# taaha-khan/2023-CompaCT-Image-Compression

Hardware: AMD Instinct MI355X
Metric: MPixels/s encode+decode, 12-bit 512x512 CT batch, bytes-exact (higher is better)
Workload: dtype u16

## Files before the change

### 2023-compact-image-compression_amd/csrc/deflate_kernels.hip

```cpp
#include <hip/hip_runtime.h>
#include <cstring>
#include <algorithm>

#include "cct_internal.h"
#include "wave_device.h"
#include "../../include/compact_hip.h"

namespace cct {
namespace {

constexpr int MIN_MATCH = 3, MAX_MATCH = 258, WSIZE = 32768;
constexpr int MIN_LOOKAHEAD = MAX_MATCH + MIN_MATCH + 1;
constexpr int MAX_DIST = WSIZE - MIN_LOOKAHEAD;
constexpr int TOO_FAR = 4096;
constexpr int BLOCK_SYMS = 16383;
constexpr int BLOCK_SYMS_ML9 = 32767;
constexpr int L_CODES = 286, D_CODES = 30, BL_CODES = 19, HEAP_SIZE = 2 * L_CODES + 1;
constexpr int END_BLOCK = 256, MAX_BITS = 15, MAX_BL_BITS = 7;
constexpr uint32_t Z_FILTERED = 1, Z_HUFFMAN_ONLY = 2, Z_RLE = 3, Z_FIXED = 4;
__host__ __device__ __forceinline__ bool short_pass(uint32_t strategy) { return strategy == Z_HUFFMAN_ONLY || strategy == Z_RLE; }

__constant__ uint8_t c_extra_lbits[29] = {0,0,0,0,0,0,0,0,1,1,1,1,2,2,2,2,3,3,3,3,4,4,4,4,5,5,5,5,0};
__constant__ uint8_t c_extra_dbits[30] = {0,0,0,0,1,1,2,2,3,3,4,4,5,5,6,6,7,7,8,8,9,9,10,10,11,11,12,12,13,13};
__constant__ uint8_t c_extra_blbits[19] = {0,0,0,0,0,0,0,0,0,0,0,0,0,0,0,0,2,3,7};
__constant__ uint8_t c_bl_order[19] = {16,17,18,0,8,7,9,6,10,5,11,4,12,3,13,2,14,1,15};
__constant__ uint8_t c_length_code[256];
__constant__ uint16_t c_base_length[29];
__constant__ uint8_t c_dist_code[512];
__constant__ uint16_t c_base_dist[30];
__constant__ uint16_t c_static_lcode[288];
__constant__ uint8_t c_static_llen[288];
__constant__ uint16_t c_static_dcode[30];

template <int HB>
__device__ __forceinline__ uint32_t hash3(uint32_t b0, uint32_t b1, uint32_t b2)
{
	constexpr int SH = (HB + 2) / 3;
	return ((b0 << (2 * SH)) ^ (b1 << SH) ^ b2) & ((1u << HB) - 1u);
}

__device__ __forceinline__ int d_code(uint32_t dist) { return dist < 256 ? c_dist_code[dist] : c_dist_code[256 + (dist >> 7)]; }

struct MatchRec { uint16_t len_full, len_quarter, dist_full, dist_quarter; };
constexpr uint32_t GEN_MAX = 16383;
__device__ __forceinline__ uint2 pack_match(uint32_t len_full, uint32_t len_quarter, uint32_t dist_full, uint32_t dist_quarter, uint32_t gen)
{
	return make_uint2((len_full | ((gen & 127u) << 9)) | ((len_quarter | ((gen >> 7) << 9)) << 16), dist_full | (dist_quarter << 16));
}
__device__ __forceinline__ MatchRec checked_match(MatchRec r, uint32_t gen, uint32_t rw, uint32_t p, uint32_t L)
{
	const uint32_t tag = (uint32_t)(r.len_full >> 9) | ((uint32_t)(r.len_quarter >> 9) << 7);
	const uint32_t lookahead = L - min(p, L);
	const uint32_t max_len = lookahead < (uint32_t)MAX_MATCH ? lookahead : (uint32_t)MAX_MATCH;
	const bool maximal = (rw >> 15) && (rw & 0x7FFFu) >= max_len && p + 2 < L;
	MatchRec o;
	const bool ok = tag == gen;
	o.len_full = ok ? (uint16_t)(r.len_full & 511u) : (uint16_t)(maximal ? max_len : 0u);
	o.len_quarter = ok ? (uint16_t)(r.len_quarter & 511u) : (uint16_t)(maximal ? max_len : 0u);
	o.dist_full = ok ? r.dist_full : (uint16_t)(maximal ? 1u : 0u);
	o.dist_quarter = ok ? r.dist_quarter : (uint16_t)(maximal ? 1u : 0u);
	return o;
}

template <bool FIRST, int HB>
__global__ void __launch_bounds__(1024) dfl_sort_pass_kernel(DeflateArgs a)
{
	constexpr int BITS = FIRST ? 8 : HB - 8, NB = 1 << BITS;
	constexpr uint32_t HMASK = (1u << HB) - 1u;
	__shared__ uint32_t offs[256];
	__shared__ uint32_t wcnt[16][NB];
	const int s = blockIdx.x;
	const uint32_t L = a.in_sizes[s];
	const uint8_t *in = a.in + (size_t)s * a.in_stride;
	const size_t base = (size_t)s * a.in_stride;
	const uint32_t npos = L >= MIN_MATCH ? L - 2 : 0;
	const uint64_t *rec_src = a.rec_in + base;
	uint64_t *rec_dst = (FIRST ? a.rec_in : a.rec_out) + base;
	const int tid = threadIdx.x, lane = tid & 63, wave = tid >> 6;
	const uint64_t lt_mask = (1ull << lane) - 1ull;
	if (tid < 256) offs[tid] = 0;
	__syncthreads();
	if (tid < NB) offs[tid] = a.sort_hist[(size_t)s * SORT_HIST + (FIRST ? 0 : 256) + tid];
	__syncthreads();
	if (wave == 0) {
		uint32_t v[4], sum = 0;
#pragma unroll
		for (int k = 0; k < 4; k++) { v[k] = offs[lane * 4 + k]; sum += v[k]; }
		uint32_t run = wave_incl_scan(sum) - sum;
#pragma unroll
		for (int k = 0; k < 4; k++) { offs[lane * 4 + k] = run; run += v[k]; }
	}
	__syncthreads();
#ifndef CCT_SORT_E
#define CCT_SORT_E 4
#endif
	constexpr int E = CCT_SORT_E;
	constexpr int ND = E / 4;
	const uint32_t last = npos ? npos - 1 : 0;
	static_assert(E % 4 == 0 && ND + 1 <= E, "pass A: whole dwords per lane, kept in ra[0 .. ND]");
#ifdef CCT_SORT_PROBE
	const bool compact = false;
#else
	const bool compact = HB == 15 && a.pos_mask != 0xFFFFFFFFu;
#endif
	const uint32_t dmax = (uint32_t)a.in_stride - 4u;
	auto fetch = [&](uint32_t tile_base, uint32_t (&ra)[E], uint32_t (&rb)[E]) {
		if (FIRST) {
#pragma unroll
			for (int d = 0; d < ND; d++) ra[d] = *reinterpret_cast<const uint32_t *>(in + min(tile_base + 256u * d + 4u * (uint32_t)lane, dmax));
			ra[ND] = *reinterpret_cast<const uint32_t *>(in + min(tile_base + 256u * ND, dmax));
#pragma unroll
			for (int e = 0; e < E; e++) rb[e] = compact ? a.run_len[base + min(tile_base + (uint32_t)(e * 64 + lane), last)] : 0u;
		} else {
#pragma unroll
			for (int e = 0; e < E; e++) {
				const uint64_t r = rec_src[min(tile_base + (uint32_t)(e * 64 + lane), last)];
				ra[e] = (uint32_t)r; rb[e] = (uint32_t)(r >> 32);
			}
		}
	};
	auto finish = [&](uint32_t tile_base, const uint32_t (&ra)[E], const uint32_t (&rb)[E], uint32_t (&h)[E], uint32_t (&p)[E]) {
#pragma unroll
		for (int e = 0; e < E; e++) {
			const uint32_t idx = tile_base + (uint32_t)(e * 64 + lane);
			if (FIRST) {
				const int la = (e & 3) * 16 + (lane >> 2);
				const uint32_t da = (uint32_t)__builtin_amdgcn_ds_bpermute(la << 2, (int)ra[e >> 2]);
				uint32_t db = (uint32_t)__builtin_amdgcn_ds_bpermute(((la + 1) & 63) << 2, (int)ra[e >> 2]);
				if ((e & 3) == 3) {
					const uint32_t nxt = (e >> 2) + 1 < ND ? (uint32_t)__builtin_amdgcn_readfirstlane((int)ra[(e >> 2) + 1 < ND ? (e >> 2) + 1 : 0]) : ra[ND];
					if (la == 63) db = nxt;
				}
				const uint32_t sh = (uint32_t)lane & 3u;
				const uint32_t w = __builtin_amdgcn_alignbyte(db, da, sh);
				const uint32_t b0 = w & 255u, b1 = (w >> 8) & 255u, b2 = (w >> 16) & 255u;
				h[e] = hash3<HB>(b0, b1, b2); p[e] = idx;
				if (compact) {
					const uint32_t b4 = (db >> (8u * sh)) & 255u;
					const uint32_t f16 = (b0 == b1 && b1 == b2) ? rb[e] : ((w >> 24) | (b4 << 8));
					h[e] |= (f16 << 15) | ((b0 >> 7) << 31); p[e] |= (b1 << 22) | (((b0 >> 5) & 3u) << 30);
				}
			}
			else { h[e] = rb[e]; p[e] = ra[e]; }
			if (idx >= npos) { h[e] = 0; p[e] = idx; }
		}
	};
	uint32_t hn[E], pn[E];
	{
		uint32_t ra[E], rb[E];
		fetch((uint32_t)(wave * 64 * E), ra, rb);
		finish((uint32_t)(wave * 64 * E), ra, rb, hn, pn);
	}
	for (uint32_t t0 = 0; t0 < npos; t0 += 1024 * E) {
		uint32_t h[E], p[E], rk[E], ra[E], rb[E];
		const uint32_t idx0 = t0 + (uint32_t)(wave * 64 * E + lane);
#pragma unroll
		for (int e = 0; e < E; e++) { h[e] = hn[e]; p[e] = pn[e]; }
		const uint32_t next_base = t0 + (uint32_t)(1024 * E + wave * 64 * E);
		fetch(next_base, ra, rb);
		for (int k = lane; k < NB; k += 64) wcnt[wave][k] = 0;
#pragma unroll
		for (int e = 0; e < E; e++) {
			const bool valid = idx0 + e * 64 < npos;
			const uint32_t d = FIRST ? (h[e] & 255u) : ((h[e] & HMASK) >> 8);
			uint64_t same = __ballot(valid);
#pragma unroll
			for (int b = 0; b < BITS; b++) {
				const bool bit = (d >> b) & 1u;
				const uint64_t bal = __ballot(bit);
				same &= bit ? bal : ~bal;
			}
			const uint32_t rank = (uint32_t)__popcll(same & lt_mask);
			uint32_t before = 0;
			if (valid) {
				before = wcnt[wave][d];
				if (rank == 0) wcnt[wave][d] = before + (uint32_t)__popcll(same);
			}
			rk[e] = before + rank;
		}
		lds_barrier();
		if (tid < NB) {
			uint32_t c[16], run = offs[tid];
#pragma unroll
			for (int w = 0; w < 16; w++) c[w] = wcnt[w][tid];
#pragma unroll
			for (int w = 0; w < 16; w++) { wcnt[w][tid] = run; run += c[w]; }
			offs[tid] = run;
		}
		lds_barrier();
#pragma unroll
		for (int e = 0; e < E; e++) asm volatile("" : "+v"(ra[e]), "+v"(rb[e]) :: "memory");
		finish(next_base, ra, rb, hn, pn);
#pragma unroll
		for (int e = 0; e < E; e++) {
			if (idx0 + e * 64 < npos) {
				const uint32_t d = FIRST ? (h[e] & 255u) : ((h[e] & HMASK) >> 8);
				const uint32_t dst = wcnt[wave][d] + rk[e];
				rec_dst[dst] = (uint64_t)p[e] | ((uint64_t)h[e] << 32);
			}
		}
	}
}

constexpr int LIGHT_STEPS = 12;

__device__ __forceinline__ bool xcd_slice(int n, int &s, uint32_t &part, uint32_t &nparts)
{
	const uint32_t lin = blockIdx.x + gridDim.x * blockIdx.y;
	const uint32_t c = lin & 7u, k = lin >> 3;
	nparts = gridDim.x;
	s = (int)(8u * (k / nparts) + c);
	part = k % nparts;
	return s < n;
}

__device__ __forceinline__ uint32_t nil_candidate(uint32_t p, uint32_t lookahead)
{
	return (lookahead < (uint32_t)MIN_LOOKAHEAD && p >= 32506u + 32768u && (p - 32506u) % 32768u == 0) ? p - 32506u : 0xFFFFFFFFu;
}


template <bool SORT, int HB>
__global__ void __launch_bounds__(256) dfl_run_len_kernel(DeflateArgs a)
{
	constexpr int NH = 256 + (1 << (HB - 8));
	__shared__ uint32_t wtot[4];
	__shared__ uint32_t hist[SORT ? NH : 1];
	if (SORT) for (int t = threadIdx.x; t < NH; t += 256) hist[t] = 0;
	__syncthreads();
	const int s = blockIdx.y;
	const uint32_t L = a.in_sizes[s];
	const uint8_t *in = a.in + (size_t)s * a.in_stride;
	uint16_t *rl = a.run_len + (size_t)s * a.in_stride;
	const int lane = threadIdx.x & 63, wave = threadIdx.x >> 6;
	const uint32_t nchunks = (L + RUNLEN_OUT - 1) / RUNLEN_OUT;
	for (uint32_t c = blockIdx.x; c < nchunks; c += gridDim.x) {
		const uint32_t c0 = c * RUNLEN_OUT;
		const uint32_t g = c0 + threadIdx.x * 8;
		uint8_t b[12];
		if (g + 12 <= L && g >= 1) {
			uint64_t w;
			__builtin_memcpy(&w, in + g, 8);
#pragma unroll
			for (int k = 0; k < 8; k++) b[k + 1] = (uint8_t)(w >> (8 * k));
			b[0] = in[g - 1];
			uint32_t w2; __builtin_memcpy(&w2, in + g + 8, 4);
			b[9] = (uint8_t)w2; b[10] = (uint8_t)(w2 >> 8); b[11] = (uint8_t)(w2 >> 16);
		} else {
#pragma unroll
			for (int k = 0; k < 12; k++) { const int64_t y = (int64_t)g - 1 + k; b[k] = (y >= 0 && y < (int64_t)L) ? in[y] : 0; }
		}
		if (SORT) {
			uint32_t hk[8], cnt = 0, h0 = 0;
			bool same = true;
#pragma unroll
			for (int k = 0; k < 8; k++) {
				const bool v = threadIdx.x * 8 + k < (uint32_t)RUNLEN_OUT && g + k + 2 < L;
				hk[k] = v ? hash3<HB>(b[k + 1], b[k + 2], b[k + 3]) : 0xFFFFFFFFu;
				if (v) { if (!cnt) h0 = hk[k]; else same &= hk[k] == h0; cnt++; }
			}
			const bool wave_same = __all(same && cnt == 8 && h0 == (uint32_t)__builtin_amdgcn_readfirstlane((int)h0));
			if (wave_same) {
				if (lane == 0) { atomicAdd(&hist[h0 & 255u], 512u); atomicAdd(&hist[256u + (h0 >> 8)], 512u); }
			} else if (same) {
				if (cnt) { atomicAdd(&hist[h0 & 255u], cnt); atomicAdd(&hist[256u + (h0 >> 8)], cnt); }
			} else {
#pragma unroll
				for (int k = 0; k < 8; k++)
					if (hk[k] != 0xFFFFFFFFu) { atomicAdd(&hist[hk[k] & 255u], 1u); atomicAdd(&hist[256u + (hk[k] >> 8)], 1u); }
			}
		}
		uint32_t chg = 0;
#pragma unroll
		for (int k = 0; k < 8; k++) chg |= (uint32_t)(b[k + 1] != b[k + 2] || g + k + 1 >= L) << k;
		uint32_t hc = chg != 0, n = hc ? (uint32_t)__ffs((int)chg) - 1u : 8u;
#pragma unroll
		for (int d = 1; d < 64; d <<= 1) {
			const uint32_t hb = (uint32_t)__shfl_down((int)hc, d, 64), nb = (uint32_t)__shfl_down((int)n, d, 64);
			if (lane + d < 64 && !hc) { n += nb; hc = hb; }
		}
		__syncthreads();
		if (lane == 0) wtot[wave] = (hc << 31) | n;
		__syncthreads();
// ... 538 lines not shown
				nxt = p + k + (uint32_t)len;
				cnt = k + 1;
			}
		}
		a.rec32[base + p] = rec;
#pragma unroll
		for (int r = 0; r < 6; r++) {
			const bool inside = nxt < blk_end;
			const int j = inside ? (int)(nxt - wb * 64) : lane;
			const uint32_t n2 = __shfl(nxt, j), c2 = __shfl(cnt, j);
			if (inside) { nxt = n2; cnt += c2; }
		}
		a.exit_pos[base + p] = (nxt - blk_end) | (cnt << 16);
	}
}

__global__ void __launch_bounds__(256) dfl_rle_rec_kernel(DeflateArgs a)
{
	const int s = blockIdx.y;
	const uint32_t L = a.in_sizes[s];
	const size_t base = (size_t)s * a.in_stride;
	const uint16_t *rl = a.run_len + base;
	const uint32_t nblk64 = (L + 63) / 64;
	const int lane = threadIdx.x & 63;
	const uint32_t lastp = L ? L - 1 : 0;
	const uint32_t wb_step = gridDim.x * (blockDim.x >> 6);
	const uint32_t wb0 = blockIdx.x * (blockDim.x >> 6) + (threadIdx.x >> 6);
	uint32_t nx = rl[min(wb0 * 64 + lane, lastp)];
	for (uint32_t wb = wb0; wb < nblk64; wb += wb_step) {
		const uint32_t p = wb * 64 + lane;
		const uint32_t blk_end = wb * 64 + 64;
		const uint32_t rw = nx;
		nx = rl[min((wb + wb_step) * 64 + lane, lastp)];
		const uint32_t rw0 = (uint32_t)__shfl((int)rw, 0);
		const bool prev_eq = p >= 2 ? (rw >> 15) != 0 : (p == 1 && (rw0 & 0x7FFFu) >= 2u);
		const uint32_t run = rw & 0x7FFFu;
		uint32_t rec = 0, nxt = blk_end, cnt = 0;
		if (p < L) {
			const bool m = prev_eq && run >= (uint32_t)MIN_MATCH;
			rec = m ? (run << 8) | (1u << 17) : 0u;
			nxt = p + (m ? run : 1u);
			cnt = 1;
		}
		a.rec32[base + p] = rec;
#pragma unroll
		for (int r = 0; r < 6; r++) {
			const bool inside = nxt < blk_end;
			const int j = inside ? (int)(nxt - wb * 64) : lane;
			const uint32_t n2 = __shfl(nxt, j), c2 = __shfl(cnt, j);
			if (inside) { nxt = n2; cnt += c2; }
		}
		a.exit_pos[base + p] = (nxt - blk_end) | (cnt << 16);
	}
}

template <uint32_t BS>
__global__ void __launch_bounds__(256) dfl_huff_symbols_kernel(DeflateArgs a)
{
	const int s = blockIdx.y;
	const uint32_t L = a.in_sizes[s];
	const size_t base = (size_t)s * a.in_stride;
	const uint32_t *in4 = reinterpret_cast<const uint32_t *>(a.in + base);
	uint4 *sym4 = reinterpret_cast<uint4 *>(a.sym + base);
	uint32_t *bend = a.blk_end + (size_t)s * a.max_blocks, *btop = a.blk_top + (size_t)s * a.max_blocks;
	if (blockIdx.x == 0 && threadIdx.x == 0) a.total_syms[s] = L;
	const uint32_t nq = (L + 3) / 4;
	for (uint32_t q = blockIdx.x * blockDim.x + threadIdx.x; q < nq; q += gridDim.x * blockDim.x) {
		const uint32_t w = in4[q], p0 = 4 * q;
		uint32_t v[4];
#pragma unroll
		for (int k = 0; k < 4; k++) {
			const uint32_t p = p0 + (uint32_t)k;
			v[k] = p < L ? (w >> (8 * k)) & 255u : 0u;
			if (p < L && p % BS == BS - 1) { bend[p / BS] = p + 1; btop[p / BS] = p; }
		}
		sym4[q] = make_uint4(v[0], v[1], v[2], v[3]);
	}
}

#ifndef CCT_WALK_T
#define CCT_WALK_T 256
#endif
constexpr int WALK_T = CCT_WALK_T;
__global__ void __launch_bounds__(WALK_T) dfl_walk_kernel(DeflateArgs a, int n)
{
	__shared__ uint32_t s_land[WALK_T];
	__shared__ uint32_t s_wsum[WALK_T / 64];
	const int s = blockIdx.x;
	(void)n;
	const uint32_t L = a.in_sizes[s];
	const size_t base = (size_t)s * a.in_stride;
	const size_t bbase = (size_t)s * dfl_blk_words(a.in_stride);
	const uint32_t *exit_rec = a.exit_pos + base;
	const int tid = threadIdx.x;
	const uint32_t seg = (((L + WALK_T - 1) / WALK_T) + 63) & ~63u;
	const uint32_t seg_end = min(L, (uint32_t)(tid + 1) * seg);
	uint32_t start = min(L, (uint32_t)tid * seg), land = start, cnt = 0;
	auto hop_through = [&]() {
		uint32_t cur = start, c = 0;
		while (cur < seg_end) { const uint32_t e = exit_rec[cur]; c += e >> 16; cur = (cur & ~63u) + 64u + (e & 0xFFFFu); }
		land = cur; cnt = c;
	};
	hop_through();
	for (;;) {
		__syncthreads();
		s_land[tid] = land;
		__syncthreads();
		const uint32_t pl = tid ? s_land[tid - 1] : 0u;
		const bool moved = tid > 0 && pl != start;
		if (!__syncthreads_or(moved)) break;
		if (moved) { start = pl; hop_through(); }
	}
	uint32_t total;
	uint32_t syms = wg_excl_scan<WALK_T / 64>(cnt, s_wsum, total);
	if (tid == 0) a.total_syms[s] = total;
	for (uint32_t cur = start; cur < seg_end;) {
		const uint32_t b = cur >> 6;
		a.blk_entry[bbase + b] = cur;
		a.blk_symbase[bbase + b] = syms;
		const uint32_t e = exit_rec[cur];
		syms += e >> 16;
		cur = (cur & ~63u) + 64u + (e & 0xFFFFu);
	}
}

template <uint32_t BS>
__global__ void __launch_bounds__(256) dfl_symbols_kernel(DeflateArgs a)
{
	const int s = blockIdx.y;
	const uint32_t L = a.in_sizes[s];
	const uint8_t *in = a.in + (size_t)s * a.in_stride;
	const size_t base = (size_t)s * a.in_stride;
	const size_t bbase = (size_t)s * dfl_blk_words(a.in_stride);
	const uint32_t nblk64 = (L + 63) / 64;
	const int lane = threadIdx.x & 63;
	uint32_t *sym = a.sym + base;
	uint32_t *bend = a.blk_end + (size_t)s * a.max_blocks, *btop = a.blk_top + (size_t)s * a.max_blocks;
	const uint32_t lazy = short_pass(a.strategy) ? 0u : 1u;
	const uint32_t wb_step = gridDim.x * (blockDim.x >> 6), wb_last = nblk64 ? nblk64 - 1 : 0;
	struct Req { uint32_t entry, symbase, rec; uint8_t lit0; };
	auto request = [&](uint32_t wb) {
		const uint32_t wbc = min(wb, wb_last), pc = min(wbc * 64 + lane, L - 1);
		return Req{a.blk_entry[bbase + wbc], a.blk_symbase[bbase + wbc], a.rec32[base + pc], in[pc]};
	};
	const uint32_t wb0 = blockIdx.x * (blockDim.x >> 6) + (threadIdx.x >> 6);
	Req nx = nblk64 ? request(wb0) : Req{0xFFFFFFFFu, 0, 0, 0};
	for (uint32_t wb = wb0; wb < nblk64; wb += wb_step) {
		const uint32_t p = wb * 64 + lane;
		const Req cur_req = nx;
		nx = request(wb + wb_step);
		const uint32_t entry = cur_req.entry, symbase = cur_req.symbase;
		uint32_t rec = cur_req.rec;
		const uint8_t lit0 = cur_req.lit0;
		if (entry == 0xFFFFFFFFu) continue;
		if (p >= L) rec = 0;
		const uint32_t k = rec & 0xFFu, len = (rec >> 8) & 0x1FFu, dist = rec >> 17;
		const uint32_t nxt = len ? p + k + len : p + 1;
		const uint32_t cnt = len ? k + 1 : 1;
		const uint64_t jump = __ballot(len != 0);
		const uint32_t nvalid = min(64u, L - wb * 64);
		uint64_t visited = 0;
		uint32_t cur = (uint32_t)__builtin_amdgcn_readfirstlane((int)(entry - wb * 64));
		while (cur < nvalid) {
			const uint64_t rest = jump >> cur;
			if (!rest) { visited |= ~0ull << cur; break; }
			const int d = __ffsll((long long)rest) - 1;
			visited |= (d >= 63 ? ~0ull : ((2ull << d) - 1ull)) << cur;
			cur = (uint32_t)__builtin_amdgcn_readlane((int)nxt, (int)cur + d) - wb * 64;
		}
		if (nvalid < 64) visited &= (1ull << nvalid) - 1ull;
		const bool mine = (visited >> lane) & 1ull;
		const uint32_t v = mine ? cnt : 0u;
		uint32_t off = symbase + wave_incl_scan(v) - v;
		if (mine) {
			if (p == L - 1) a.postloop_lit[s] = 1;
			for (uint32_t t = 0; t < (len ? k : 1u); t++, off++) {
				sym[off] = t ? in[p + t] : lit0;
				if (off % BS == BS - 1) { bend[off / BS] = p + t + 1; btop[off / BS] = p + t + lazy; }
			}
			if (len) {
				sym[off] = (len - MIN_MATCH) | (dist << 16);
				if (off % BS == BS - 1) { bend[off / BS] = p + k + len; btop[off / BS] = p + k + lazy; }
			}
		}
	}
}

struct TreeScratch {
	uint16_t freq[HEAP_SIZE], dad[HEAP_SIZE], len[HEAP_SIZE], code[L_CODES + 2];
	uint16_t dfreq[2 * D_CODES + 1], ddad[2 * D_CODES + 1], dlen[2 * D_CODES + 1], dcode[D_CODES + 2];
	uint16_t bfreq[2 * BL_CODES + 1], bdad[2 * BL_CODES + 1], blen[2 * BL_CODES + 1], bcode[BL_CODES + 1];
	alignas(16) uint32_t heap[HEAP_SIZE + 11];
	uint32_t bl_count[MAX_BITS + 1];
	uint16_t next_code[MAX_BITS + 1];
	int heap_len, heap_max, max_code, overflow, lmax, dmax;
	uint32_t opt_len, static_len, dyn_body_bits;
	uint32_t hdr_bits[160];
	uint32_t hdr_nbits;
	int ntok, btype, max_blindex;
	uint8_t extra_l[29], extra_d[30], extra_bl[19], bl_order[19];
	__device__ __forceinline__ uint32_t *hist_l() { return heap; }
	__device__ __forceinline__ uint32_t *hist_d() { return heap + L_CODES + 2; }
	__device__ __forceinline__ uint8_t *length_code() { return reinterpret_cast<uint8_t *>(dad); }
	__device__ __forceinline__ uint8_t *dist_code() { return reinterpret_cast<uint8_t *>(dad) + 256; }
	__device__ __forceinline__ uint16_t *tok() { return dad; }
};
// ... 747 lines not shown
					nb = t_llen[lsym];
					int extra = t_extra_l[code];
					if (extra) { bits |= (uint64_t)(lc - t_base_length[code]) << nb; nb += extra; }
					dist--;
					code = dist < 256 ? t_dist_code[dist] : t_dist_code[256 + (dist >> 7)];
					bits |= (uint64_t)t_dcode[code] << nb;
					nb += t_dlen[code];
					extra = t_extra_d[code];
					if (extra) { bits |= (uint64_t)(dist - t_base_dist[code]) << nb; nb += extra; }
				}
			} else if (i == bm.nsym) {
				bits = t_lcode[END_BLOCK];
				nb = t_llen[END_BLOCK];
			}
			const uint32_t q = ltot >> 6, r = ltot & 63;
			const uint64_t lo = bits << r, hi = r ? bits >> (64 - r) : 0ull;
#pragma unroll
			for (int j = 0; j < EMIT_LIMBS; j++) {
				if (q == (uint32_t)j) acc[j] |= lo;
				if (q + 1 == (uint32_t)j) acc[j] |= hi;
			}
			ltot += (uint32_t)nb;
		}
		const uint32_t inc = wave_incl_scan(ltot);
		if (lane == 63) wsum[par][wave] = inc;
		__syncthreads();
		uint32_t wb = 0, tot = 0;
		for (int w = 0; w < 4; w++) { if (w < wave) wb += wsum[par][w]; tot += wsum[par][w]; }
		uint32_t *wbf = wbuf[par];
		const uint32_t lbit = (uint32_t)(run & 31) + wb + inc - ltot;
		if (ltot) {
			const uint32_t w0 = lbit >> 5, sh = lbit & 31, nw = (sh + ltot + 31) >> 5;
#pragma unroll
			for (int j = 0; j <= 2 * EMIT_LIMBS; j++) {
				const uint32_t aj = j < 2 * EMIT_LIMBS ? (uint32_t)(acc[j >> 1] >> (32 * (j & 1))) : 0u;
				const uint32_t ap = j > 0 ? (uint32_t)(acc[(j - 1) >> 1] >> (32 * ((j - 1) & 1))) : 0u;
				const uint32_t w = (uint32_t)((((uint64_t)aj << 32) | ap) >> (32 - sh));
				if ((uint32_t)j < nw && w) atomicOr(&wbf[w0 + j], w);
			}
		}
		__syncthreads();
		const uint32_t nwords = ((uint32_t)(run & 31) + tot + 31) >> 5;
		const uint64_t gw = run >> 5;
		for (uint32_t k = threadIdx.x; k < nwords; k += blockDim.x) {
			const uint32_t w = wbf[k];
			wbf[k] = 0;
			if (k == 0 || k == nwords - 1) { if (w) atomicOr(&words[gw + k], w); }
			else words[gw + k] = w;
		}
		run += tot;
	}
}

__global__ void __launch_bounds__(256) dfl_pack_offsets_kernel(const uint32_t *sizes, int n, uint64_t *offsets, int exact)
{
	__shared__ uint64_t wsum[4];
	const int t = threadIdx.x, lane = t & 63, wave = t >> 6;
	uint64_t carry = 0;
	for (int base = 0; base < n; base += 256) {
		const int i = base + t;
		const uint32_t sz = i < n ? sizes[i] : 0u;
		const uint64_t v = exact ? sz : (uint64_t)((sz + 15u) & ~15u);
		const uint64_t inc = wave_incl_scan(v);
		if (lane == 63) wsum[wave] = inc;
		__syncthreads();
		uint64_t wb = 0, tot = 0;
		for (int w = 0; w < 4; w++) { if (w < wave) wb += wsum[w]; tot += wsum[w]; }
		if (i < n) offsets[i] = carry + wb + inc - v;
		carry += tot;
		__syncthreads();
	}
	if (t == 0) offsets[n] = carry;
}
__global__ void __launch_bounds__(256) dfl_pack_kernel(const uint8_t *src, size_t stride, const uint32_t *sizes,
                                                       const uint64_t *offsets, uint8_t *dst)
{
	const int s = blockIdx.y;
	const uint32_t n16 = (sizes[s] + 15u) >> 4;
	const uint4 *in = reinterpret_cast<const uint4 *>(src + (size_t)s * stride);
	uint4 *out = reinterpret_cast<uint4 *>(dst + offsets[s]);
	for (uint32_t i = blockIdx.x * blockDim.x + threadIdx.x; i < n16; i += gridDim.x * blockDim.x) out[i] = in[i];
}

__global__ void dfl_offsets2_kernel(DeflateArgs a, int n)
{
	const size_t per = dfl_blk_words(a.in_stride);
	for (size_t i = blockIdx.x * (size_t)blockDim.x + threadIdx.x; i < (size_t)n * per; i += (size_t)gridDim.x * blockDim.x)
		a.blk_entry[i] = 0xFFFFFFFFu;
}

__global__ void dfl_offsets_kernel(DeflateArgs a, int n)
{
	if (blockIdx.x == 0) {
		for (int s = threadIdx.x; s < n; s += blockDim.x) { a.postloop_lit[s] = 0; a.heavy_count[s] = 0; a.deep_count[s] = 0; a.run_end_count[s] = 0; }
		if (threadIdx.x == 0) *a.gen = *a.gen % GEN_MAX + 1u;
	}
	const size_t nrc = dfl_hist_words((size_t)n, (size_t)a.run_chunks);
	for (size_t t = (size_t)blockIdx.x * blockDim.x + threadIdx.x; t < nrc; t += (size_t)gridDim.x * blockDim.x) a.sort_hist[t] = 0;
}

constexpr uint32_t CLEAR_SLACK = 64;
__device__ __forceinline__ size_t clear_bytes(const DeflateArgs &a, int s)
{
	const size_t L = a.in_sizes[s];
	const size_t bound = a.block_syms == (uint32_t)BLOCK_SYMS ? L + (L >> 12) + (L >> 14) + (L >> 25) + 13
	                                                          : L + ((L + 7) >> 3) + ((L + 63) >> 6) + 5 + 6;
	return min(a.out_stride, (13 + bound + CLEAR_SLACK + 15) & ~(size_t)15);
}
template <typename W>
__global__ void __launch_bounds__(256) dfl_clear_kernel(DeflateArgs a)
{
	const int s = blockIdx.y;
	const size_t units = clear_bytes(a, s) / sizeof(W);
	W *out = reinterpret_cast<W *>(a.out + (size_t)s * a.out_stride);
	W zero{};
	for (size_t i = blockIdx.x * (size_t)blockDim.x + threadIdx.x; i < units; i += (size_t)gridDim.x * blockDim.x) out[i] = zero;
}
static void launch_clear(const DeflateArgs &a, int n, hipStream_t st)
{
	if (a.out_stride % 16 == 0 && (uintptr_t)a.out % 16 == 0) hipLaunchKernelGGL(dfl_clear_kernel<uint4>, dim3(16, n), dim3(256), 0, st, a);
	else hipLaunchKernelGGL(dfl_clear_kernel<uint32_t>, dim3(32, n), dim3(256), 0, st, a);
}

}

bool deflate_level_args(int level, DeflateArgs &a)
{
	static const uint32_t T[6][5] = {
		{4, 4, 16, 16, 0x5E}, {8, 16, 32, 32, 0x5E}, {8, 16, 128, 128, 0x9C},
		{8, 32, 128, 256, 0xDA}, {32, 128, 258, 1024, 0xDA}, {32, 258, 258, 4096, 0xDA},
	};
	if (level < 4 || level > 9) return false;
	const uint32_t *t = T[level - 4];
	a.good = t[0]; a.max_lazy = t[1]; a.nice = t[2]; a.max_chain = t[3]; a.zlib_flg = t[4];
	return true;
}

bool deflate_strategy_args(int level, int strategy, DeflateArgs &a)
{
	if (strategy < 0 || strategy > (int)Z_FIXED) return false;
	a.strategy = (uint32_t)strategy;
	a.min_len = strategy == (int)Z_FILTERED ? 6u : (uint32_t)MIN_MATCH;
	if (short_pass((uint32_t)strategy)) {
		if (level < 1 || level > 9) return false;
		a.good = a.max_lazy = a.nice = a.max_chain = 0;
		a.zlib_flg = 0x01;
		return true;
	}
	if (!deflate_level_args(level, a)) return false;
	if (strategy == (int)Z_FIXED) a.zlib_flg = 0x01;
	return true;
}

bool deflate_mem_level_args(int mem_level, DeflateArgs &a)
{
	if (mem_level != 8 && mem_level != 9) return false;
	a.hash_bits = (uint32_t)mem_level + 7u;
	a.block_syms = (1u << (mem_level + 6)) - 1u;
	return true;
}

static int g_tree_cus = 0;
hipError_t deflate_init_tables()
{
	uint8_t length_code[256]; uint16_t base_length[29]; uint8_t dist_code[512]; uint16_t base_dist[30];
	uint16_t static_lcode[288]; uint8_t static_llen[288]; uint16_t static_dcode[30];
	static const int xl[29] = {0,0,0,0,0,0,0,0,1,1,1,1,2,2,2,2,3,3,3,3,4,4,4,4,5,5,5,5,0};
	static const int xd[30] = {0,0,0,0,1,1,2,2,3,3,4,4,5,5,6,6,7,7,8,8,9,9,10,10,11,11,12,12,13,13};
	int length = 0, code, n, dist = 0;
	for (code = 0; code < 28; code++) {
		base_length[code] = (uint16_t)length;
		for (n = 0; n < (1 << xl[code]); n++) length_code[length++] = (uint8_t)code;
	}
	length_code[length - 1] = (uint8_t)code;
	base_length[28] = 0;
	for (code = 0; code < 16; code++) {
		base_dist[code] = (uint16_t)dist;
		for (n = 0; n < (1 << xd[code]); n++) dist_code[dist++] = (uint8_t)code;
	}
	dist >>= 7;
	for (; code < 30; code++) {
		base_dist[code] = (uint16_t)(dist << 7);
		for (n = 0; n < (1 << (xd[code] - 7)); n++) dist_code[256 + dist++] = (uint8_t)code;
	}
	uint16_t bl_count[16] = {0}, next_code[16];
	n = 0;
	while (n <= 143) { static_llen[n++] = 8; bl_count[8]++; }
	while (n <= 255) { static_llen[n++] = 9; bl_count[9]++; }
	while (n <= 279) { static_llen[n++] = 7; bl_count[7]++; }
	while (n <= 287) { static_llen[n++] = 8; bl_count[8]++; }
	unsigned c = 0;
	for (int bits = 1; bits <= 15; bits++) { c = (c + bl_count[bits - 1]) << 1; next_code[bits] = (uint16_t)c; }
	auto rev = [](unsigned v, int len) { unsigned r = 0; do { r |= v & 1; v >>= 1; r <<= 1; } while (--len > 0); return r >> 1; };
	for (n = 0; n < 288; n++) static_lcode[n] = (uint16_t)rev(next_code[static_llen[n]]++, static_llen[n]);
	for (n = 0; n < 30; n++) static_dcode[n] = (uint16_t)rev((unsigned)n, 5);
	hipError_t e;
	if ((e = hipMemcpyToSymbol(HIP_SYMBOL(c_length_code), length_code, sizeof length_code)) != hipSuccess) return e;
	if ((e = hipMemcpyToSymbol(HIP_SYMBOL(c_base_length), base_length, sizeof base_length)) != hipSuccess) return e;
	if ((e = hipMemcpyToSymbol(HIP_SYMBOL(c_dist_code), dist_code, sizeof dist_code)) != hipSuccess) return e;
	if ((e = hipMemcpyToSymbol(HIP_SYMBOL(c_base_dist), base_dist, sizeof base_dist)) != hipSuccess) return e;
	if ((e = hipMemcpyToSymbol(HIP_SYMBOL(c_static_lcode), static_lcode, sizeof static_lcode)) != hipSuccess) return e;
	if ((e = hipMemcpyToSymbol(HIP_SYMBOL(c_static_llen), static_llen, sizeof static_llen)) != hipSuccess) return e;
	if ((e = hipMemcpyToSymbol(HIP_SYMBOL(c_static_dcode), static_dcode, sizeof static_dcode)) != hipSuccess) return e;
	int dev;
	if ((e = hipGetDevice(&dev)) != hipSuccess) return e;
	if ((e = hipDeviceGetAttribute(&g_tree_cus, hipDeviceAttributeMultiprocessorCount, dev)) != hipSuccess) return e;
	return hipFuncSetAttribute(reinterpret_cast<const void *>(dfl_tree_kernel<16>), hipFuncAttributeMaxDynamicSharedMemorySize,
	                           (int)(16 * sizeof(TreeScratch)));
}

constexpr int TREE_WAVES16_MIN_SLICES = 128;
template <int WAVES>
static void launch_tree_waves(const DeflateArgs &a, int n, hipStream_t st)
{
	hipLaunchKernelGGL(dfl_tree_kernel<WAVES>, dim3(n, (a.max_blocks + WAVES - 1) / WAVES), dim3(64 * WAVES),
	                   WAVES * sizeof(TreeScratch), st, a, (uint32_t)g_tree_cus);
}
static void launch_tree(const DeflateArgs &a0, int n, hipStream_t st)
{
	DeflateArgs a = a0;
	if (a.tree_waves == 0 && (n < TREE_WAVES16_MIN_SLICES || n > g_tree_cus)) a.tree_waves = 1;
	if (a.tree_waves != 1) launch_tree_waves<16>(a, n, st);
	if (a.tree_waves != 16) launch_tree_waves<1>(a, n, st);
}

static hipError_t launch_deflate_short(const DeflateArgs &a, int n, hipStream_t st)
{
	const bool ml9 = a.block_syms == (uint32_t)BLOCK_SYMS_ML9;
	const int gx = (int)std::min<size_t>(64, (a.in_stride + 255) / 256);
	launch_clear(a, n, st);
	if (a.strategy == Z_RLE) {
		hipLaunchKernelGGL((dfl_run_len_kernel<false, 15>), dim3(gx, n), dim3(256), 0, st, a);
		hipLaunchKernelGGL(dfl_rle_rec_kernel, dim3(gx, n), dim3(256), 0, st, a);
		hipLaunchKernelGGL(dfl_offsets2_kernel, dim3(256), dim3(256), 0, st, a, n);
		hipLaunchKernelGGL(dfl_walk_kernel, dim3(n), dim3(WALK_T), 0, st, a, n);
		if (ml9) hipLaunchKernelGGL(dfl_symbols_kernel<BLOCK_SYMS_ML9>, dim3(gx, n), dim3(256), 0, st, a);
		else hipLaunchKernelGGL(dfl_symbols_kernel<BLOCK_SYMS>, dim3(gx, n), dim3(256), 0, st, a);
	} else {
		if (ml9) hipLaunchKernelGGL(dfl_huff_symbols_kernel<BLOCK_SYMS_ML9>, dim3(gx, n), dim3(256), 0, st, a);
		else hipLaunchKernelGGL(dfl_huff_symbols_kernel<BLOCK_SYMS>, dim3(gx, n), dim3(256), 0, st, a);
	}
	hipLaunchKernelGGL(dfl_adler_kernel, dim3(n), dim3(256), 0, st, a);
	launch_tree(a, n, st);
	hipLaunchKernelGGL(dfl_layout_kernel, dim3(n), dim3(64), 0, st, a, n);
	hipLaunchKernelGGL(dfl_emit_kernel, dim3(a.max_blocks, n), dim3(256), 0, st, a);
	return hipGetLastError();
}

hipError_t launch_deflate(const DeflateArgs &a, int n, hipStream_t st, hipStream_t side, const hipEvent_t *ev)
{
	hipError_t e;
	const bool ml9 = a.hash_bits == 16;
	if ((a.hash_bits != 15 && !ml9) || a.block_syms != (uint32_t)(ml9 ? BLOCK_SYMS_ML9 : BLOCK_SYMS)) return hipErrorInvalidValue;
	if (ml9 && a.pos_mask != 0xFFFFFFFFu) return hipErrorInvalidValue;
	if ((a.out_stride & 3) || ((uintptr_t)a.out & 3)) return hipErrorInvalidValue;
	if (a.tree_waves != 0 && a.tree_waves != 1 && a.tree_waves != 16) return hipErrorInvalidValue;
	if (short_pass(a.strategy)) return launch_deflate_short(a, n, st);
	hipLaunchKernelGGL(dfl_offsets_kernel, dim3(64), dim3(256), 0, st, a, n);
	const int gx = (int)std::min<size_t>(64, (a.in_stride + 255) / 256);
	if (ml9) {
		hipLaunchKernelGGL((dfl_run_len_kernel<true, 16>), dim3(gx, n), dim3(256), 0, st, a);
		hipLaunchKernelGGL((dfl_sort_pass_kernel<true, 16>), dim3(n), dim3(1024), 0, st, a);
		hipLaunchKernelGGL((dfl_sort_pass_kernel<false, 16>), dim3(n), dim3(1024), 0, st, a);
	} else {
		hipLaunchKernelGGL((dfl_run_len_kernel<true, 15>), dim3(gx, n), dim3(256), 0, st, a);
		hipLaunchKernelGGL((dfl_sort_pass_kernel<true, 15>), dim3(n), dim3(1024), 0, st, a);
		hipLaunchKernelGGL((dfl_sort_pass_kernel<false, 15>), dim3(n), dim3(1024), 0, st, a);
	}
	const bool fork = side != nullptr && ev != nullptr;
	hipStream_t s2 = fork ? side : st;
	if (fork) {
		if ((e = hipEventRecord(ev[0], st)) != hipSuccess) return e;
		if ((e = hipStreamWaitEvent(s2, ev[0], 0)) != hipSuccess) return e;
	}
	hipLaunchKernelGGL(dfl_run_lists_kernel, dim3(a.run_chunks, n), dim3(256), 0, s2, a);
	hipLaunchKernelGGL(dfl_run_info_kernel, dim3(8, n), dim3(256), 0, s2, a);
	launch_clear(a, n, s2);
	hipLaunchKernelGGL(dfl_offsets2_kernel, dim3(256), dim3(256), 0, s2, a, n);
	const int n8 = (n + 7) & ~7;
	const int gm_cap = a.pos_mask == COMPACT_POS_MASK ? std::max(DFL_MATCH_GRID, 256 / std::max(1, n8 / 8)) : 2048;
	const int gm = (int)std::min<size_t>(gm_cap, (a.in_stride + 255) / 256);
	if (a.max_chain < 16 || a.max_chain > 4096 || a.nice < 16 || a.nice > (uint32_t)MAX_MATCH) return hipErrorInvalidValue;
	const bool ql = (a.max_chain >> 2) <= (uint32_t)LIGHT_STEPS;
	if (a.pos_mask == COMPACT_POS_MASK) {
		if (ql) hipLaunchKernelGGL((dfl_match_kernel<true, true>), dim3(gm, n8), dim3(256), 0, st, a, n);
		else hipLaunchKernelGGL((dfl_match_kernel<true, false>), dim3(gm, n8), dim3(256), 0, st, a, n);
	} else if (a.pos_mask == 0xFFFFFFFFu) {
		if (ql) hipLaunchKernelGGL((dfl_match_kernel<false, true>), dim3(gm, n8), dim3(256), 0, st, a, n);
		else hipLaunchKernelGGL((dfl_match_kernel<false, false>), dim3(gm, n8), dim3(256), 0, st, a, n);
	} else return hipErrorInvalidValue;
	if (fork) {
		if ((e = hipEventRecord(ev[1], st)) != hipSuccess) return e;
		if ((e = hipEventRecord(ev[2], s2)) != hipSuccess) return e;
		if ((e = hipStreamWaitEvent(s2, ev[1], 0)) != hipSuccess) return e;
		if ((e = hipStreamWaitEvent(st, ev[2], 0)) != hipSuccess) return e;
	}
	hipLaunchKernelGGL(dfl_match_heavy_kernel, dim3(gx, n8), dim3(256), 0, s2, a, n);
	hipLaunchKernelGGL(dfl_adler_kernel, dim3(n), dim3(256), 0, s2, a);
	hipLaunchKernelGGL(dfl_match_run_kernel, dim3(gx, n8), dim3(256), 0, st, a, n);
	if (fork) {
		if ((e = hipEventRecord(ev[3], s2)) != hipSuccess) return e;
		if ((e = hipStreamWaitEvent(st, ev[3], 0)) != hipSuccess) return e;
	}
	hipLaunchKernelGGL(dfl_rec_kernel, dim3(gx, n), dim3(256), 0, st, a);
	hipLaunchKernelGGL(dfl_walk_kernel, dim3(n), dim3(WALK_T), 0, st, a, n);
	if (ml9) hipLaunchKernelGGL(dfl_symbols_kernel<BLOCK_SYMS_ML9>, dim3(gx, n), dim3(256), 0, st, a);
	else hipLaunchKernelGGL(dfl_symbols_kernel<BLOCK_SYMS>, dim3(gx, n), dim3(256), 0, st, a);
	launch_tree(a, n, st);
	hipLaunchKernelGGL(dfl_layout_kernel, dim3(n), dim3(64), 0, st, a, n);
	hipLaunchKernelGGL(dfl_emit_kernel, dim3(a.max_blocks, n), dim3(256), 0, st, a);
	return hipGetLastError();
}

__global__ void __launch_bounds__(256) dfl_pack_exact_kernel(const uint8_t *src, size_t stride, const uint32_t *sizes,
                                                             const uint64_t *offsets, uint8_t *dst)
{
	const int s = blockIdx.y;
	const uint32_t nbytes = sizes[s];
	const uint8_t *in = src + (size_t)s * stride;
	uint8_t *out = dst + offsets[s];
	const uint32_t head = min((uint32_t)(-(uintptr_t)out & 3u), nbytes);
	const uint32_t nd = (nbytes - head) >> 2;
	const uint32_t tid = blockIdx.x * blockDim.x + threadIdx.x, nth = gridDim.x * blockDim.x;
	const uint32_t *in32 = reinterpret_cast<const uint32_t *>(in);
	uint32_t *out32 = reinterpret_cast<uint32_t *>(out + head);
	const uint32_t sh = 8u * head, up = head ? 1u : 0u;
	for (uint32_t j = tid; j < nd; j += nth) {
		const uint64_t pair = ((uint64_t)in32[j + up] << 32) | in32[j];
		out32[j] = (uint32_t)(pair >> sh);
	}
	const uint32_t tail0 = head + 4u * nd;
	if (tid < head) out[tid] = in[tid];
	if (tid < nbytes - tail0) out[tail0 + tid] = in[tail0 + tid];
}

hipError_t launch_pack(const uint8_t *src, size_t stride, const uint32_t *sizes, int n, uint64_t *offsets, uint8_t *dst,
                       int exact, hipStream_t st)
{
	hipLaunchKernelGGL(dfl_pack_offsets_kernel, dim3(1), dim3(256), 0, st, sizes, n, offsets, exact);
	if (exact) hipLaunchKernelGGL(dfl_pack_exact_kernel, dim3(32, n), dim3(256), 0, st, src, stride, sizes, offsets, dst);
	else hipLaunchKernelGGL(dfl_pack_kernel, dim3(16, n), dim3(256), 0, st, src, stride, sizes, offsets, dst);
	return hipGetLastError();
}

}
```

Before: 18350.

## Stage radix-sort scatter through LDS so global writes are tile-ordered and coalesced

The sort pass kernel now ranks each tile's records into a shared-memory staging buffer ordered by digit, then reads them back contiguously and writes each to global at digit base plus local index. This replaces the random per-record global scatter with mostly consecutive stores within each digit bucket, aiming for better write coalescing. It costs extra LDS (the stage buffer, which also holds the per-wave counts), an extra cross-wave scan and more barriers, and it could affect occupancy alongside a co-resident inflate workgroup. A probe template variant is added behind a compile flag.

```diff
diff --git a/2023-compact-image-compression_amd/csrc/deflate_kernels.hip b/2023-compact-image-compression_amd/csrc/deflate_kernels.hip
--- a/2023-compact-image-compression_amd/csrc/deflate_kernels.hip
+++ b/2023-compact-image-compression_amd/csrc/deflate_kernels.hip
@@ -62,13 +62,15 @@
 	return o;
 }
 
-template <bool FIRST, int HB>
+template <bool FIRST, int HB, bool PROBE = false>
 __global__ void __launch_bounds__(1024) dfl_sort_pass_kernel(DeflateArgs a)
 {
 	constexpr int BITS = FIRST ? 8 : HB - 8, NB = 1 << BITS;
 	constexpr uint32_t HMASK = (1u << HB) - 1u;
 	__shared__ uint32_t offs[256];
-	__shared__ uint32_t wcnt[16][NB];
+	__shared__ uint32_t tstart[256];
+	__shared__ uint32_t gbase[256];
+	__shared__ uint32_t wsum[4];
 	const int s = blockIdx.x;
 	const uint32_t L = a.in_sizes[s];
 	const uint8_t *in = a.in + (size_t)s * a.in_stride;
@@ -95,14 +97,14 @@
 #define CCT_SORT_E 4
 #endif
 	constexpr int E = CCT_SORT_E;
+	__shared__ uint64_t stage[1024 * E];
+	static_assert(sizeof(uint32_t) * 16 * NB <= sizeof(stage), "the digit counts live inside the stage");
+	static_assert(sizeof(stage) + sizeof(offs) + sizeof(tstart) + sizeof(gbase) + sizeof(wsum) <= 163840 - 122336, "sort + INFLATE workgroup on one CU");
+	uint32_t (*wcnt)[NB] = reinterpret_cast<uint32_t (*)[NB]>(stage);
 	constexpr int ND = E / 4;
 	const uint32_t last = npos ? npos - 1 : 0;
 	static_assert(E % 4 == 0 && ND + 1 <= E, "pass A: whole dwords per lane, kept in ra[0 .. ND]");
-#ifdef CCT_SORT_PROBE
-	const bool compact = false;
-#else
 	const bool compact = HB == 15 && a.pos_mask != 0xFFFFFFFFu;
-#endif
 	const uint32_t dmax = (uint32_t)a.in_stride - 4u;
 	auto fetch = [&](uint32_t tile_base, uint32_t (&ra)[E], uint32_t (&rb)[E]) {
 		if (FIRST) {
@@ -179,26 +181,63 @@
 			rk[e] = before + rank;
 		}
 		lds_barrier();
+		uint32_t total = 0, incl = 0;
 		if (tid < NB) {
-			uint32_t c[16], run = offs[tid];
-#pragma unroll
-			for (int w = 0; w < 16; w++) c[w] = wcnt[w][tid];
-#pragma unroll
-			for (int w = 0; w < 16; w++) { wcnt[w][tid] = run; run += c[w]; }
-			offs[tid] = run;
+#pragma unroll
+			for (int w0 = 0; w0 < 16; w0 += 8) {
+				uint32_t c[8];
+#pragma unroll
+				for (int w = 0; w < 8; w++) c[w] = wcnt[w0 + w][tid];
+#pragma unroll
+				for (int w = 0; w < 8; w++) { wcnt[w0 + w][tid] = total; total += c[w]; }
+			}
+			incl = wave_incl_scan(total);
+			if (lane == 63) wsum[wave] = incl;
+		}
+		lds_barrier();
+		if (tid < NB) {
+			uint32_t start = incl - total;
+#pragma unroll
+			for (int w = 0; w < NB / 64; w++) start += w < wave ? wsum[w] : 0u;
+			const uint32_t o = offs[tid];
+			tstart[tid] = start;
+			gbase[tid] = o - start;
+			offs[tid] = o + total;
+		}
+#pragma unroll
+		for (int e = 0; e < E; e++) {
+			const uint32_t d = FIRST ? (h[e] & 255u) : ((h[e] & HMASK) >> 8);
+			rk[e] += wcnt[wave][d];
+		}
+		lds_barrier();
+#pragma unroll
+		for (int e = 0; e < E; e++) {
+			const uint32_t d = FIRST ? (h[e] & 255u) : ((h[e] & HMASK) >> 8);
+			rk[e] += tstart[d];
+		}
+#pragma unroll
+		for (int e = 0; e < E; e++)
+			if (idx0 + e * 64 < npos) stage[rk[e]] = (uint64_t)p[e] | ((uint64_t)h[e] << 32);
+		lds_barrier();
+		const uint32_t in_tile = min(npos - t0, (uint32_t)(1024 * E));
+		uint64_t r[E];
+		uint32_t dst[E];
+#pragma unroll
+		for (int e = 0; e < E; e++) {
+			const uint32_t j = min((uint32_t)(e * 1024 + tid), in_tile - 1u);
+			r[e] = stage[j];
+			const uint32_t hw = (uint32_t)(r[e] >> 32);
+			const uint32_t d = FIRST ? (hw & 255u) : ((hw & HMASK) >> 8);
+			dst[e] = gbase[d] + j;
+			if (PROBE) dst[e] = min(t0 + j + (dst[e] >> 31), last);
 		}
 		lds_barrier();
 #pragma unroll
 		for (int e = 0; e < E; e++) asm volatile("" : "+v"(ra[e]), "+v"(rb[e]) :: "memory");
 		finish(next_base, ra, rb, hn, pn);
 #pragma unroll
-		for (int e = 0; e < E; e++) {
-			if (idx0 + e * 64 < npos) {
-				const uint32_t d = FIRST ? (h[e] & 255u) : ((h[e] & HMASK) >> 8);
-				const uint32_t dst = wcnt[wave][d] + rk[e];
-				rec_dst[dst] = (uint64_t)p[e] | ((uint64_t)h[e] << 32);
-			}
-		}
+		for (int e = 0; e < E; e++)
+			if ((uint32_t)(e * 1024 + tid) < in_tile) rec_dst[dst[e]] = r[e];
 	}
 }
 
@@ -2038,6 +2077,11 @@
 		hipLaunchKernelGGL((dfl_sort_pass_kernel<false, 16>), dim3(n), dim3(1024), 0, st, a);
 	} else {
 		hipLaunchKernelGGL((dfl_run_len_kernel<true, 15>), dim3(gx, n), dim3(256), 0, st, a);
+#ifdef CCT_SORT_PROBE
+		hipLaunchKernelGGL((dfl_sort_pass_kernel<true, 15, true>), dim3(n), dim3(1024), 0, st, a);
+		hipLaunchKernelGGL((dfl_sort_pass_kernel<true, 15>), dim3(n), dim3(1024), 0, st, a);
+		hipLaunchKernelGGL((dfl_sort_pass_kernel<false, 15, true>), dim3(n), dim3(1024), 0, st, a);
+#endif
 		hipLaunchKernelGGL((dfl_sort_pass_kernel<true, 15>), dim3(n), dim3(1024), 0, st, a);
 		hipLaunchKernelGGL((dfl_sort_pass_kernel<false, 15>), dim3(n), dim3(1024), 0, st, a);
 	}
```

Result: no change. 18370 (median of 5 runs) (+0.1%).

## Cache walk hop chain in LDS and drop separate blk_entry clear kernel

Applied to the files above, without the earlier changes.

The walk kernel now records each hop's position and running symbol prefix in shared memory, up to a per-thread cap. When a segment's start moves during the fixpoint iteration, it re-walks only until it meets a cached position, then fixes up the prefixes by a delta instead of re-hopping the whole segment. The final pass writes entries and symbol bases from the cache and fills skipped blocks with the sentinel itself, so the separate dfl_offsets2 clear kernel and its launches are removed. This trades about 60KB of LDS per block, which limits occupancy, for fewer global exit_rec reads and one fewer launch.

```diff
diff --git a/2023-compact-image-compression_amd/csrc/deflate_kernels.hip b/2023-compact-image-compression_amd/csrc/deflate_kernels.hip
--- a/2023-compact-image-compression_amd/csrc/deflate_kernels.hip
+++ b/2023-compact-image-compression_amd/csrc/deflate_kernels.hip
@@ -903,8 +903,11 @@
 #define CCT_WALK_T 256
 #endif
 constexpr int WALK_T = CCT_WALK_T;
+constexpr int WALK_CAP = (60 * 1024) / (8 * WALK_T);
+constexpr uint32_t WALK_NONE = 0xFFFFFFFFu;
 __global__ void __launch_bounds__(WALK_T) dfl_walk_kernel(DeflateArgs a, int n)
 {
+	__shared__ uint32_t s_pos[WALK_CAP * WALK_T], s_pre[WALK_CAP * WALK_T];
 	__shared__ uint32_t s_land[WALK_T];
 	__shared__ uint32_t s_wsum[WALK_T / 64];
 	const int s = blockIdx.x;
@@ -916,13 +919,35 @@
 	const int tid = threadIdx.x;
 	const uint32_t seg = (((L + WALK_T - 1) / WALK_T) + 63) & ~63u;
 	const uint32_t seg_end = min(L, (uint32_t)(tid + 1) * seg);
-	uint32_t start = min(L, (uint32_t)tid * seg), land = start, cnt = 0;
-	auto hop_through = [&]() {
-		uint32_t cur = start, c = 0;
+	const uint32_t kb = (uint32_t)tid * (seg >> 6), nblk64 = (L + 63) / 64;
+	const uint32_t nb = min(seg >> 6, nblk64 > kb ? nblk64 - kb : 0u);
+	const uint32_t ncap = min(nb, (uint32_t)WALK_CAP);
+	uint32_t *const t_pos = s_pos + tid, *const t_pre = s_pre + tid;
+	uint32_t start = min(L, (uint32_t)tid * seg), land = start, cnt = 0, bias = 0, tail_pos = start, tail_pre = 0;
+	auto walk = [&](const bool restart) {
+		uint32_t cur = start, c = 0, k_next = 0;
+		const uint32_t k0 = (start >> 6) - kb;
+		while (cur < seg_end) {
+			const uint32_t k = (cur >> 6) - kb;
+			if (k >= (uint32_t)WALK_CAP) break;
+			for (; k_next < k; k_next++) t_pos[k_next * WALK_T] = WALK_NONE;
+			if (restart && t_pos[k * WALK_T] == cur) {
+				const uint32_t delta = c - (t_pre[k * WALK_T] + bias);
+				for (uint32_t j = k0; j < k; j++) t_pre[j * WALK_T] -= delta;
+				bias += delta; cnt += delta; tail_pre += delta;
+				return;
+			}
+			t_pos[k * WALK_T] = cur; t_pre[k * WALK_T] = c - bias; k_next = k + 1;
+			const uint32_t e = exit_rec[cur];
+			c += e >> 16;
+			cur = (cur & ~63u) + 64u + (e & 0xFFFFu);
+		}
+		for (; k_next < ncap; k_next++) t_pos[k_next * WALK_T] = WALK_NONE;
+		tail_pos = cur; tail_pre = c;
 		while (cur < seg_end) { const uint32_t e = exit_rec[cur]; c += e >> 16; cur = (cur & ~63u) + 64u + (e & 0xFFFFu); }
 		land = cur; cnt = c;
 	};
-	hop_through();
+	walk(false);
 	for (;;) {
 		__syncthreads();
 		s_land[tid] = land;
@@ -930,19 +955,27 @@
 		const uint32_t pl = tid ? s_land[tid - 1] : 0u;
 		const bool moved = tid > 0 && pl != start;
 		if (!__syncthreads_or(moved)) break;
-		if (moved) { start = pl; hop_through(); }
+		if (moved) { start = pl; walk(true); }
 	}
 	uint32_t total;
-	uint32_t syms = wg_excl_scan<WALK_T / 64>(cnt, s_wsum, total);
+	const uint32_t syms = wg_excl_scan<WALK_T / 64>(cnt, s_wsum, total);
 	if (tid == 0) a.total_syms[s] = total;
-	for (uint32_t cur = start; cur < seg_end;) {
+	uint32_t *const entry = a.blk_entry + bbase, *const symbase = a.blk_symbase + bbase;
+	for (uint32_t k = 0; k < ncap; k++) {
+		const uint32_t pos = t_pos[k * WALK_T];
+		entry[kb + k] = pos;
+		if (pos != WALK_NONE) symbase[kb + k] = syms + t_pre[k * WALK_T] + bias;
+	}
+	uint32_t b_next = kb + ncap, sy = syms + tail_pre;
+	for (uint32_t cur = tail_pos; cur < seg_end;) {
 		const uint32_t b = cur >> 6;
-		a.blk_entry[bbase + b] = cur;
-		a.blk_symbase[bbase + b] = syms;
+		for (; b_next < b; b_next++) entry[b_next] = WALK_NONE;
+		entry[b] = cur; symbase[b] = sy; b_next = b + 1;
 		const uint32_t e = exit_rec[cur];
-		syms += e >> 16;
+		sy += e >> 16;
 		cur = (cur & ~63u) + 64u + (e & 0xFFFFu);
 	}
+	for (; b_next < kb + nb; b_next++) entry[b_next] = WALK_NONE;
 }
 
 template <uint32_t BS>
@@ -1856,13 +1889,6 @@
 	for (uint32_t i = blockIdx.x * blockDim.x + threadIdx.x; i < n16; i += gridDim.x * blockDim.x) out[i] = in[i];
 }
 
-__global__ void dfl_offsets2_kernel(DeflateArgs a, int n)
-{
-	const size_t per = dfl_blk_words(a.in_stride);
-	for (size_t i = blockIdx.x * (size_t)blockDim.x + threadIdx.x; i < (size_t)n * per; i += (size_t)gridDim.x * blockDim.x)
-		a.blk_entry[i] = 0xFFFFFFFFu;
-}
-
 __global__ void dfl_offsets_kernel(DeflateArgs a, int n)
 {
 	if (blockIdx.x == 0) {
@@ -2006,7 +2032,6 @@
 	if (a.strategy == Z_RLE) {
 		hipLaunchKernelGGL((dfl_run_len_kernel<false, 15>), dim3(gx, n), dim3(256), 0, st, a);
 		hipLaunchKernelGGL(dfl_rle_rec_kernel, dim3(gx, n), dim3(256), 0, st, a);
-		hipLaunchKernelGGL(dfl_offsets2_kernel, dim3(256), dim3(256), 0, st, a, n);
 		hipLaunchKernelGGL(dfl_walk_kernel, dim3(n), dim3(WALK_T), 0, st, a, n);
 		if (ml9) hipLaunchKernelGGL(dfl_symbols_kernel<BLOCK_SYMS_ML9>, dim3(gx, n), dim3(256), 0, st, a);
 		else hipLaunchKernelGGL(dfl_symbols_kernel<BLOCK_SYMS>, dim3(gx, n), dim3(256), 0, st, a);
@@ -2050,7 +2075,6 @@
 	hipLaunchKernelGGL(dfl_run_lists_kernel, dim3(a.run_chunks, n), dim3(256), 0, s2, a);
 	hipLaunchKernelGGL(dfl_run_info_kernel, dim3(8, n), dim3(256), 0, s2, a);
 	launch_clear(a, n, s2);
-	hipLaunchKernelGGL(dfl_offsets2_kernel, dim3(256), dim3(256), 0, s2, a, n);
 	const int n8 = (n + 7) & ~7;
 	const int gm_cap = a.pos_mask == COMPACT_POS_MASK ? std::max(DFL_MATCH_GRID, 256 / std::max(1, n8 / 8)) : 2048;
 	const int gm = (int)std::min<size_t>(gm_cap, (a.in_stride + 255) / 256);
```

After: 18470 before, 18430 after. Within noise of the previous version (-0.2%).
